# Illumina/Pisces

Measured on AMD Instinct MI355X. Metric: candidate loci/s at 500x depth, higher is better.
Workload: dtype int32 counts + f64 likelihoods; 1 GPU; BASELINE config 2: synthetic 100000 loci x 500x amplicon pileup, SNV-only, gVCF, per GPU per step; device-resident packed tuples; depth=500, ring_batches=6, tile_loci=56, parallelism=interval-shard x1

## Files before the change

### include/pisces_hip.h

```cpp
#ifndef PISCES_HIP_H
#define PISCES_HIP_H

#include <stdint.h>

#ifdef __cplusplus
extern "C" {
#endif

#define PISCES_HIP_ABI_VERSION 8

#define PISCES_OK                 0
#define PISCES_E_INVALID_ARG     -1
#define PISCES_E_BUFFER_TOO_SMALL -2
#define PISCES_E_DEVICE          -3
#define PISCES_E_UNMAPPED_BASE   -4
#define PISCES_E_UNSUPPORTED     -5
#define PISCES_E_STATE           -6
#define PISCES_E_INTERNAL        -7

enum { PISCES_ALLELE_A = 0, PISCES_ALLELE_G = 1, PISCES_ALLELE_C = 2, PISCES_ALLELE_T = 3,
       PISCES_ALLELE_N = 4, PISCES_ALLELE_DEL = 5, PISCES_NUM_ALLELE_TYPES = 6 };
enum { PISCES_DIR_FORWARD = 0, PISCES_DIR_REVERSE = 1, PISCES_DIR_STITCHED = 2, PISCES_NUM_DIRECTIONS = 3 };
enum { PISCES_CAT_SNV = 0, PISCES_CAT_INSERTION = 1, PISCES_CAT_DELETION = 2, PISCES_CAT_MNV = 3,
       PISCES_CAT_REFERENCE = 4 };
// ... 145 lines not shown
    const uint8_t* directions;
    const uint8_t* deletion_directions;
} PiscesReadBatch;
#define PISCES_DIR_UNTRACKED 255

typedef struct PiscesCandidate {
    int32_t position;
    int32_t category;
    int32_t ref_len, alt_len;
    int32_t support_by_dir[3];
    int32_t well_anchored_by_dir[3];
    uint8_t open_left, open_right;
    uint8_t pad[2];
    int64_t allele_offset;
} PiscesCandidate;

typedef struct PiscesHip PiscesHip;

int32_t pisces_hip_default_config(PiscesHipConfig* cfg);
int32_t pisces_hip_create(const PiscesHipConfig* cfg, int32_t device, PiscesHip** out);
int32_t pisces_hip_device_count(void);
int32_t pisces_hip_destroy(PiscesHip* h);
int64_t pisces_hip_trim_memory(void);
const char* pisces_hip_last_error(const PiscesHip* h);
int32_t pisces_hip_abi_version(void);

int32_t pisces_hip_set_reference(PiscesHip* h, const uint8_t* upper_bases, int64_t length);

int32_t pisces_hip_set_intervals(PiscesHip* h, const int32_t* starts, const int32_t* ends, int32_t n);

int32_t pisces_hip_set_owned_range(PiscesHip* h, int32_t lo, int32_t hi);

int32_t pisces_hip_add_reads(PiscesHip* h, const PiscesReadBatch* batch);
int32_t pisces_hip_stage_reads(PiscesHip* h, int32_t n_reads, int64_t n_cigar_ops, int64_t n_bases, int32_t with_directions,
                               int32_t with_deletion_directions, PiscesReadBatch* views);
int32_t pisces_hip_add_device_reads(PiscesHip* h, const PiscesReadBatch* device_batch, int64_t n_cigar_ops, int64_t n_bases);
int32_t pisces_hip_add_observations(PiscesHip* h, const int32_t* positions, const uint32_t* tuples, int64_t n);
int32_t pisces_hip_flush(PiscesHip* h, int32_t up_to_position, PiscesCalledAllele* out,
                         int64_t capacity, int64_t* n_out);
int32_t pisces_hip_flush_ex(PiscesHip* h, int32_t up_to_position, PiscesCalledAllele* out, int64_t capacity, int64_t* n_out,
                            int32_t* cand_index_out, PiscesCandidate* cand_out, int64_t cand_capacity, int64_t* n_cand,
                            uint8_t* alleles_out, int64_t allele_capacity, int64_t* allele_bytes);
int32_t pisces_hip_flush_begin(PiscesHip* h, int32_t up_to_position);
int32_t pisces_hip_flush_end(PiscesHip* h, PiscesCalledAllele* out, int64_t capacity, int64_t* n_out);
int32_t pisces_hip_flush_end_ex(PiscesHip* h, PiscesCalledAllele* out, int64_t capacity, int64_t* n_out, int32_t* cand_index_out,
                                PiscesCandidate* cand_out, int64_t cand_capacity, int64_t* n_cand, uint8_t* alleles_out,
// ... 194 lines not shown
```

### pisces_amd/_native.py

```python
import ctypes as C
import os

from . import _abi

_HERE = os.path.dirname(os.path.abspath(__file__))
LIB_PATH = os.environ.get("PISCES_HIP_LIB") or os.path.join(_HERE, "libpisceship.so")

EXPORTS = [
    "pisces_hip_abi_version", "pisces_hip_default_config", "pisces_hip_create", "pisces_hip_destroy", "pisces_hip_trim_memory",
    "pisces_hip_last_error", "pisces_hip_set_reference", "pisces_hip_set_intervals", "pisces_hip_add_reads", "pisces_hip_stage_reads", "pisces_hip_flush_begin", "pisces_hip_flush_end",
    "pisces_hip_add_observations", "pisces_hip_flush", "pisces_hip_get_counts", "pisces_hip_add_gapped_mnv_ref",
    "pisces_hip_get_candidates", "pisces_hip_stats", "pisces_hip_call_tiles", "pisces_hip_accumulate_tiles",
    "pisces_hip_synchronize", "pisces_hip_last_kernel_ms", "pisces_hip_expand_reads", "pisces_hip_device_totals",
    "pisces_hip_set_timing", "pisces_hip_kernel_time", "pisces_hip_set_chain_timing", "pisces_hip_chain_time", "pisces_hip_flush_ex", "pisces_hip_probe_read_bandwidth",
    "pisces_hip_vcf_default_config", "pisces_hip_format_vcf", "pisces_hip_format_vcf_padded", "pisces_hip_find_candidates", "pisces_hip_call_tiles_batched",
    "pisces_hip_find_indel_candidates", "pisces_hip_compact_records", "pisces_hip_bgzf_scan", "pisces_hip_bgzf_inflate",
    "pisces_hip_balanced_tile_loci", "pisces_hip_bam_decode", "pisces_hip_bam_fetch", "pisces_hip_bam_chain_mode", "pisces_hip_add_decoded_reads", "pisces_hip_find_candidates_device", "pisces_hip_get_base_quality_sums", "pisces_hip_get_gapped_mnv_ref", "pisces_hip_comm_unique_id", "pisces_hip_comm_init", "pisces_hip_reduce_summary", "pisces_hip_comm_destroy",
    "pisces_hip_add_candidates", "pisces_hip_set_forced_alleles", "pisces_hip_host_time", "pisces_hip_set_owned_range", "pisces_hip_bam_fetch_directions", "pisces_hip_call_tiles_graph_build", "pisces_hip_call_tiles_graph_launch", "pisces_hip_mark", "pisces_hip_marked_ms",
    "pisces_hip_flush_end_ex", "pisces_hip_device_count", "pisces_hip_flush_view", "pisces_hip_flush_end_view", "pisces_hip_transfer_bytes",
    "pisces_hip_add_device_reads", "pisces_hip_get_stream", "pisces_hip_comm_library", "pisces_hip_comm_ranks", "pisces_hip_set_known_variants", "pisces_hip_set_exclude_mnvs_from_collapsing", "pisces_hip_set_exact_total_called", "pisces_hip_reallocate_failed_mnvs", "pisces_hip_set_genotypes", "pisces_hip_diploid_genotype_qscore",
    "pisces_hip_adaptive_default_params", "pisces_hip_set_adaptive_params", "pisces_hip_get_posteriors", "pisces_hip_posteriors_view", "pisces_hip_set_posteriors_buffer",
    "pisces_hip_compact_posteriors", "pisces_hip_set_genotypes_adaptive", "pisces_hip_adaptive_genotype_qscore", "pisces_hip_format_vcf_ex", "pisces_hip_format_vcf_padded_ex",
    "pisces_hip_amplicon_bias", "pisces_hip_set_amplicon_bias_filter", "pisces_hip_add_reads_amplicons", "pisces_hip_add_device_reads_amplicons",
    "pisces_hip_get_amplicon_counts", "pisces_hip_bam_fetch_amplicons", "pisces_hip_amplicon_name_count", "pisces_hip_get_amplicon_name",
    "pisces_hip_intern_amplicon_name",
    "pisces_hip_exact_span_direction", "pisces_hip_set_coverage_method", "pisces_hip_get_spanning_read_counts",
    "pisces_hip_format_vcf_device",
]


class PiscesHipError(RuntimeError):
    def __init__(self, code, message):
# ... 7 lines not shown
    spec = importlib.util.find_spec("torch")
    if spec is None or not spec.origin:
        return
    cand = os.path.join(os.path.dirname(spec.origin), "lib", "libamdhip64.so")
    if os.path.exists(cand):
        C.CDLL(cand, mode=C.RTLD_GLOBAL)


def _load():
    _share_hip_runtime_with_torch()
    if not os.path.exists(LIB_PATH):
        raise ImportError(
            f"{LIB_PATH} is missing: the HIP extension has not been built. Run `python -c 'import __graft_entry__ as g; "
            "g.build()'` (needs hipcc). pisces_amd has no CPU fallback.")
    lib = C.CDLL(LIB_PATH)
    i32, i64, vp = C.c_int32, C.c_int64, C.c_void_p
    P = C.POINTER
    sig = {
        "pisces_hip_abi_version": (i32, []),
        "pisces_hip_default_config": (i32, [P(_abi.PiscesHipConfig)]),
        "pisces_hip_create": (i32, [P(_abi.PiscesHipConfig), i32, P(vp)]),
        "pisces_hip_destroy": (i32, [vp]),
        "pisces_hip_trim_memory": (C.c_int64, []),
        "pisces_hip_last_error": (C.c_char_p, [vp]),
        "pisces_hip_set_reference": (i32, [vp, vp, i64]),
        "pisces_hip_set_intervals": (i32, [vp, vp, vp, i32]),
        "pisces_hip_add_reads": (i32, [vp, P(_abi.PiscesReadBatch)]),
        "pisces_hip_add_device_reads": (i32, [vp, P(_abi.PiscesReadBatch), i64, i64]),
        "pisces_hip_reallocate_failed_mnvs": (i32, [vp, i64, vp, i64, vp, i64, i32, vp, i64, P(i64), vp, i64, P(i64), vp, i64, P(i64)]),
        "pisces_hip_set_genotypes": (i32, [P(_abi.PiscesHipConfig), P(_abi.PiscesGenotypeAllele), i32, vp, i64]),
        "pisces_hip_diploid_genotype_qscore": (i32, [i32, i32, i32, i32, i32]),
        "pisces_hip_adaptive_default_params": (i32, [P(_abi.PiscesAdaptiveParams)]),
        "pisces_hip_set_adaptive_params": (i32, [vp, P(_abi.PiscesAdaptiveParams)]),
        "pisces_hip_get_posteriors": (i32, [vp, vp, i64, P(i64)]),
        "pisces_hip_posteriors_view": (i32, [vp, P(vp), P(i64)]),
        "pisces_hip_set_posteriors_buffer": (i32, [vp, vp, i64]),
        "pisces_hip_compact_posteriors": (i32, [vp, vp, vp, i32, vp, vp, i32, vp]),
        "pisces_hip_set_genotypes_adaptive": (i32, [P(_abi.PiscesHipConfig), P(_abi.PiscesAdaptiveParams), P(_abi.PiscesGenotypeAllele), i32, vp, i64, vp]),
        "pisces_hip_adaptive_genotype_qscore": (i32, [P(_abi.PiscesAdaptiveParams), i32, i32, i32, i32, P(i32), P(i32), P(C.c_float)]),
        "pisces_hip_amplicon_bias": (i32, [P(i32), P(i32), i32, C.c_float, P(C.c_double)]),
        "pisces_hip_set_amplicon_bias_filter": (i32, [vp, C.c_float]),
        "pisces_hip_add_reads_amplicons": (i32, [vp, P(_abi.PiscesReadBatch), vp]),
        "pisces_hip_add_device_reads_amplicons": (i32, [vp, P(_abi.PiscesReadBatch), i64, i64, vp]),
        "pisces_hip_get_amplicon_counts": (i32, [vp, i32, i32, vp, vp, vp]),
        "pisces_hip_stage_reads": (i32, [vp, i32, i64, i64, i32, i32, P(_abi.PiscesReadBatch)]),
        "pisces_hip_flush_begin": (i32, [vp, i32]),
# ... 84 lines not shown
```

### pisces_amd/csrc/device_math.hip.h

```cpp
#pragma once
#include <hip/hip_runtime.h>
#include <stdint.h>

#include "../../include/pisces_hip.h"
#include "poisson_core.h"

namespace pisces {

struct DeviceParams {
    int32_t min_bq, noise_level, max_vq, min_vq, vq_filter, min_cov, low_depth_filter;
    int32_t min_gq, max_gq, low_gq_filter, sb_model, filter_single_strand, include_ref, emit_zero_cov;
    int32_t rmxn_max_len, rmxn_min_rep;
    float min_freq, vf_filter, gt_min_freq, target_lod, nocall_thr, rmxn_freq_limit;
    double sb_threshold;
    double err_q;
    double err_sb;
    double ln10;
    unsigned long long* totals;
    const double* q_to_p_lut;
    int32_t q_to_p_n;
    const double* gq_tail;
    int32_t gq_tail_a, gq_tail_cov;
    int32_t refs_only;
    int32_t variants_only;
    const int16_t* vq_tab;
    const double* sb_tab;
    const double* sb0_tab;
    const int16_t* gq_cap;
    int32_t vq_tab_k, sb_tab_k, tab_cov;
    const uint32_t* dirty_bits;
    int32_t dirty_first, dirty_n;
    int32_t* folded_out;
    int32_t folded_first, folded_n;
};

__device__ __forceinline__ bool locus_is_dirty(const DeviceParams& P, int pos)
{
    if (!P.dirty_bits) return false;
    const unsigned rel = (unsigned)(pos - P.dirty_first);
    return rel < (unsigned)P.dirty_n && ((P.dirty_bits[rel >> 5] >> (rel & 31u)) & 1u) != 0u;
}


__device__ __forceinline__ double ln_lower_bound(double r) { return (double)ilogb(r) * 0.6931471805; }

__device__ inline double poisson_cdf_sb(double num_occurrences, double expected)
{
    const double a = (double)(int)(num_occurrences + 1.0), x = expected;
    if (x > 0.0 && a >= 1.0 && 2.0 * x <= a) {
        const double r = a / x;
        if (a * (ln_lower_bound(r) - 1.0) + x > 51.0) return 1.0;
        if (a * (log(r) - 1.0) + x > 51.0) return 1.0;
    }
    return incomplete_gamma_function(a, x);
}


// ... 406 lines not shown
        if (nonAlleleObservationsF >= expectedNonAllelObservationsF) { gq = P.min_gq; return true; }
        return false;
    }
    double qScore = fmin((double)P.max_gq, (double)variantQ);
    qScore = fmax(qScore, (double)P.min_gq);
    gq = (int32_t)rint(qScore);
    return true;
}

struct AlleleTables {
    int32_t vq;
    double sb[3];
    int32_t gq_cap;
    int32_t gq_idx;
    uint32_t have;
};
__device__ __forceinline__ bool tables_complete(const DeviceParams& P) { return P.vq_tab && P.sb_tab && P.sb0_tab && P.gq_cap; }

__device__ __forceinline__ AlleleTables request_allele_tables(bool isRef, int32_t support, int32_t total, int32_t refsup, const int32_t cov[3],
                                                              const int32_t sup[3], const DeviceParams& P)
{
    AlleleTables t;
    const uint32_t tab_cov = (uint32_t)P.tab_cov;
    const bool vq_in = support > 0 && total > 0 && support < P.vq_tab_k && total < P.tab_cov;
    const int16_t vq_v = P.vq_tab[vq_in ? (uint32_t)support * tab_cov + (uint32_t)total : 0u];
    const int s2 = sup[2] / 2, c2 = cov[2] / 2;
    const int ss[3] = {sup[0] + sup[1] + sup[2], sup[0] + s2, sup[1] + s2};
    const int cc[3] = {cov[0] + cov[1] + cov[2], cov[0] + c2, cov[1] + c2};
    double sb_v[3];
    uint32_t have = vq_in ? 1u : 0u;
#pragma unroll
    for (int w = 0; w < 3; w++) {
        const bool zero = ss[w] == 0;
        const bool in = zero ? (P.sb_model != PISCES_SB_POISSON && cc[w] >= 0 && cc[w] < P.tab_cov)
                             : (ss[w] > 0 && ss[w] < P.sb_tab_k && cc[w] >= 0 && cc[w] < P.tab_cov);
        const double* base = zero ? P.sb0_tab : P.sb_tab;
        const uint32_t idx = in ? (zero ? (uint32_t)cc[w] : (uint32_t)ss[w] * tab_cov + (uint32_t)cc[w]) : 0u;
        sb_v[w] = base[idx];
        have |= in ? (2u << w) : 0u;
    }
    t.gq_idx = somatic_gq_index(somatic_genotype(isRef, total, support, refsup, P), total, support, P);
    const int16_t gq_v = P.gq_cap[t.gq_idx >= 0 ? t.gq_idx : 0];
    t.vq = vq_v;
    t.sb[0] = sb_v[0]; t.sb[1] = sb_v[1]; t.sb[2] = sb_v[2];
    t.gq_cap = gq_v;
    t.have = have;
    return t;
}

__device__ __forceinline__ bool poisson_qscore_try(int32_t callCount, int32_t coverage, const DeviceParams& P, const AlleleTables& t, int32_t& vq)
{
    if ((callCount <= 0) || (coverage <= 0)) { vq = 0; return true; }
    if (t.have & 1u) { vq = t.vq; return true; }
    const double lambda = P.err_q * coverage;
    if (P.max_vq <= 110 && callCount >= 3 && (double)callCount >= 2.0 * lambda) {
        const double km1 = callCount - 1;
        const double need = ((double)P.max_vq + 1.0) * 0.23025850929940458 + 1e-3;
        if (km1 * (ln_ratio_lower_bound(km1, lambda) - 1.0) >= need) { vq = P.max_vq; return true; }
    }
    return false;
}

__device__ __forceinline__ bool sb_stats_try(int32_t support, int32_t coverage, const DeviceParams& P, bool have, double value, SbStats& st)
{
    st.support = (double)support;
    st.coverage = (double)coverage;
    if (support == 0) {
        if (P.sb_model == PISCES_SB_POISSON) {
            st.false_pos = 1;
            st.var_gt_zero = 0;
            return true;
        }
        if (!have) return false;
        st.var_gt_zero = value;
        st.false_pos = 1 - st.var_gt_zero;
        return true;
    }
    if (have) {
        st.var_gt_zero = value;
    } else {
        const double a = (double)support, x = (double)coverage * P.err_sb;
        if (!(x > 0.0 && 2.0 * x <= a && a * (ln_ratio_lower_bound(a, x) - 1.0) + x > 51.0)) return false;
        st.var_gt_zero = 1.0;
    }
    st.false_pos = fmax(0.0, 1 - st.var_gt_zero);
    return true;
}

__device__ __forceinline__ bool strand_bias_try(const int32_t cov[3], const int32_t sup[3], const DeviceParams& P, const AlleleTables& t,
                                                double& bias_score, int& acceptable, int& var_both, int& cov_both)
{
    const int s2 = sup[2] / 2, c2 = cov[2] / 2;
    const int sf = sup[0] + s2, sr = sup[1] + s2, cf = cov[0] + c2, cr = cov[1] + c2;
    SbStats overall, fwd, rev;
    const bool ok0 = sb_stats_try(sup[0] + sup[1] + sup[2], cov[0] + cov[1] + cov[2], P, (t.have & 2u) != 0, t.sb[0], overall);
    const bool ok1 = sb_stats_try(sf, cf, P, (t.have & 4u) != 0, t.sb[1], fwd);
    const bool ok2 = sb_stats_try(sr, cr, P, (t.have & 8u) != 0, t.sb[2], rev);
    double forwardBias = 0.0, reverseBias = 0.0;
    if (!(fwd.false_pos == 0.0 && rev.false_pos == 0.0 && overall.var_gt_zero > 0.0)) {
        forwardBias = (fwd.var_gt_zero * rev.false_pos) / overall.var_gt_zero;
        reverseBias = (rev.var_gt_zero * fwd.false_pos) / overall.var_gt_zero;
        if (overall.var_gt_zero == 0) {
            forwardBias = 1;
            reverseBias = 1;
        }
    }
    double score = forwardBias > reverseBias ? forwardBias : reverseBias;
    cov_both = (cf > 0) && (cr > 0);
    var_both = (sf > 0) && (sr > 0);
    if (!cov_both) score = 0;
    bias_score = score;
    acceptable = score < P.sb_threshold;
    return ok0 && ok1 && ok2;
}

__device__ __noinline__ int32_t poisson_qscore_out_of_line(int32_t callCount, int32_t coverage, double err, int32_t max_vq, double ln10)
{
    const QParams q = {max_vq, ln10};
    return poisson_qscore_core(callCount, coverage, err, q);
}
// ... 80 lines not shown
```

### pisces_amd/csrc/kernels.hip.h

```cpp
#pragma once
#include <hip/hip_runtime.h>
#include <stdint.h>

#include "device_math.hip.h"
#include "genotype_core.h"

namespace pisces {

constexpr int kBlock = 256;
constexpr int kTile = 64;
constexpr int kFolded = 18;
constexpr int kUnroll = 8;
constexpr int kSlotsPerTile = 4 * kTile;
#ifndef PISCES_TOTAL_SHARDS
#define PISCES_TOTAL_SHARDS 64
#endif
constexpr int kTotalShards = PISCES_TOTAL_SHARDS;
constexpr int kTotalStride = 16;
constexpr int kRefMargin = 32;
constexpr int kRefWin = kTile + 2 * kRefMargin;
constexpr int kWaveRows = 32;
constexpr int kWaveRow = kTile;
constexpr int kWaveRegion = kWaveRows * kWaveRow;
constexpr int kQLutLds = 128;
// ... 707 lines not shown
__global__ __launch_bounds__(256) void build_vq_tab_kernel(int16_t* __restrict__ tab, int32_t n_k, int32_t n_cov, DeviceParams P)
{
    const int64_t i = (int64_t)blockIdx.x * blockDim.x + threadIdx.x;
    if (i >= (int64_t)n_k * n_cov) return;
    tab[i] = (int16_t)poisson_qscore((int32_t)(i / n_cov), (int32_t)(i % n_cov), P);
}
__global__ __launch_bounds__(256) void build_sb_tab_kernel(double* __restrict__ tab, double* __restrict__ tab0, int32_t n_k, int32_t n_cov, DeviceParams P)
{
    const int64_t i = (int64_t)blockIdx.x * blockDim.x + threadIdx.x;
    if (i >= (int64_t)n_k * n_cov) return;
    const int k = (int)(i / n_cov), cov = (int)(i % n_cov);
    tab[i] = k >= 1 ? fmax(0.0, poisson_cdf_sb((double)k - 1, (double)cov * P.err_sb)) : 0.0;
    if (k == 0) tab0[cov] = pow(1 - P.err_sb, (double)cov);
}
__global__ __launch_bounds__(256) void build_gq_cap_kernel(int16_t* __restrict__ tab, const double* __restrict__ gq_tail, int32_t n_a, int32_t n_cov, DeviceParams P)
{
    const int64_t i = (int64_t)blockIdx.x * blockDim.x + threadIdx.x;
    if (i >= (int64_t)n_a * n_cov) return;
    if (i < n_cov) { tab[i] = 0; return; }
    double rawQ = p_to_q(q_to_p_int(P.max_vq, P) + gq_tail[i]);
    double qScore = fmin((double)P.max_gq, rawQ);
    qScore = fmax(qScore, (double)P.min_gq);
    tab[i] = (int16_t)rint(qScore);
}

__global__ __launch_bounds__(64) void totals_collect_kernel(unsigned long long* __restrict__ shards, unsigned long long* __restrict__ out_host, int reset)
{
    const int l = threadIdx.x;
    if (l < 4) {
        unsigned long long v = 0;
        for (int sh = 0; sh < kTotalShards; sh++) v += shards[sh * kTotalStride + l];
        out_host[l] = v;
    }
    if (reset)
        for (int i = l; i < kTotalShards * kTotalStride; i += 64) shards[i] = 0ull;
    __threadfence_system();
}

__global__ __launch_bounds__(256) void read_probe_kernel(const u32x4* __restrict__ p, int64_t n4, uint32_t* __restrict__ sink)
{
    uint32_t acc = 0;
    const int64_t stride = (int64_t)gridDim.x * blockDim.x * 8;
    for (int64_t i = (int64_t)blockIdx.x * blockDim.x * 8 + threadIdx.x; i < n4; i += stride) {
        u32x4 v[8];
#pragma unroll
        for (int u = 0; u < 8; u++) {
// ... 808 lines not shown
```

### pisces_amd/csrc/pisces_hip.hip

```cpp
#include <hip/hip_runtime.h>
#include <hip/hip_ext.h>
#include <dlfcn.h>
#include <link.h>

#include <algorithm>
#include <array>
#include <cctype>
#include <memory>
#include <cmath>
#include <cstdio>
#include <cstdlib>
#include <cstring>
#include <deque>
#include <ctime>
#include <map>
#include <set>
#include <string>
#include <atomic>
#include <chrono>
#include <mutex>
#include <thread>
#include <unordered_map>
#include <unordered_set>
#include <vector>
// ... 263 lines not shown
    std::unordered_map<std::string, int32_t> amp_name_id;
    bool exact_on = false;
    bool exact_l0_set = false;
    DeviceBuf<int32_t> d_exact_words;
    DeviceBuf<int32_t> d_exact_extra, d_exact_spans, d_exact_out;
    DeviceBuf<PiscesTile> d_tiles_x;
    DeviceBuf<PiscesTileResult> d_tr_x;
    DeviceBuf<PiscesCalledAllele> d_rec_x;
    DeviceBuf<int32_t> d_cnt_x, d_off_x;
    int32_t* h_cnt_x = nullptr;
    bool tables_shareable = false;
    bool poisoned = false;
    std::string poison_why;
    uint8_t* h_prep = nullptr;
    DeviceBuf<double> d_qlut;
    DeviceBuf<ulonglong2> d_bq_lut;
    DeviceBuf<unsigned long long> d_sumq_fix;
    DeviceBuf<double> d_sumq;
    DeviceBuf<double> d_gq_tail;
    DeviceBuf<int16_t> d_vq_tab;
    DeviceBuf<double> d_sb_tab;
    DeviceBuf<double> d_sb0_tab;
    DeviceBuf<int16_t> d_gq_cap;
    DeviceBuf<DeviceParams> d_params;
    int n_cus = 256;
    void* comm = nullptr;
    int comm_world = 1;
    DeviceBuf<long long> d_summary;
    DeviceBuf<int32_t> d_offsets;
    DeviceBuf<PiscesCalledAllele> d_compact;
    DeviceBuf<PiscesGenotypePosteriors> d_post, d_post_compact;
    int kernel_variant = 4;
    std::string err;

    DeviceBuf<uint8_t> d_ref;
    std::vector<uint8_t> h_ref;
    int64_t ref_len = 0;
    DeviceBuf<DevCandidate> d_cands;
    DeviceBuf<uint8_t> d_alleles;
    DeviceBuf<PiscesCalledAllele> d_cand_records;
    DeviceBuf<uint8_t> d_cand_callable;
    int32_t* h_counts = nullptr;
    size_t h_counts_cap = 0;

    std::map<int32_t, BlockObs> blocks;
    int32_t last_block_key_cache = 0;
// ... 313 lines not shown
    P.min_bq = c.min_base_call_quality;
    P.noise_level = c.noise_level;
    P.max_vq = c.max_variant_qscore;
    P.min_vq = c.min_variant_qscore;
    P.vq_filter = c.variant_qscore_filter;
    P.min_cov = c.min_coverage;
    P.low_depth_filter = c.low_depth_filter;
    P.min_gq = c.min_genotype_qscore;
    P.max_gq = c.max_genotype_qscore;
    P.low_gq_filter = c.low_gq_filter;
    P.sb_model = c.strand_bias_model;
    P.filter_single_strand = c.filter_single_strand;
    P.include_ref = c.include_reference_calls;
    P.emit_zero_cov = c.emit_zero_coverage_refs;
    P.rmxn_max_len = c.rmxn_max_repeat_length;
    P.rmxn_min_rep = c.rmxn_min_repetitions;
    P.min_freq = c.min_frequency;
    P.vf_filter = c.variant_freq_filter;
    P.gt_min_freq = c.genotype_min_freq_filter;
    P.target_lod = c.target_lod_frequency;
    P.nocall_thr = c.no_call_filter_threshold;
    P.rmxn_freq_limit = c.rmxn_frequency_limit;
    P.sb_threshold = (double)c.strand_bias_threshold;
    P.err_q = std::pow(10.0, -1 * (double)c.noise_level / 10.0);
    P.err_sb = std::pow(10.0, (double)((float)(-1 * c.noise_level) / 10.0f));
    P.ln10 = std::log(10.0);
    P.totals = nullptr;
    P.q_to_p_lut = nullptr;
    P.q_to_p_n = 0;
    P.gq_tail = nullptr;
    P.gq_tail_a = 0;
    P.gq_tail_cov = 0;
    P.refs_only = c.call_mnvs ? 1 : 0;
    P.variants_only = 0;
    P.vq_tab = nullptr;
    P.sb_tab = nullptr;
    P.sb0_tab = nullptr;
    P.gq_cap = nullptr;
    P.vq_tab_k = P.sb_tab_k = P.tab_cov = 0;
    P.dirty_bits = nullptr;
    P.dirty_first = P.dirty_n = 0;
    P.folded_out = nullptr;
    P.folded_first = P.folded_n = 0;
    return P;
}

template <typename R, typename F>
static R abi_guard(PiscesHip* h, F&& body)
{
    try {
        return body();
    } catch (const std::exception& e) {
        return (R)fail(h, PISCES_E_INTERNAL, std::string("exception inside the library: ") + e.what());
    } catch (...) {
        return (R)fail(h, PISCES_E_INTERNAL, "unknown exception inside the library");
    }
}

namespace {
struct TableSet {
    PiscesHipConfig cfg;
    int device = 0;
    DeviceBuf<double> gq_tail, sb_tab, sb0_tab;
    DeviceBuf<int16_t> vq_tab, gq_cap;
};
std::mutex g_tables_mu;
std::vector<TableSet*>& table_cache() { static std::vector<TableSet*>* v = new std::vector<TableSet*>(); return *v; }
TableSet* take_tables(const PiscesHipConfig& cfg, int device)
{
    std::lock_guard<std::mutex> lock(g_tables_mu);
    auto& v = table_cache();
    for (size_t i = 0; i < v.size(); i++)
        if (v[i]->device == device && std::memcmp(&v[i]->cfg, &cfg, sizeof(cfg)) == 0) {
            TableSet* t = v[i];
            v.erase(v.begin() + (std::ptrdiff_t)i);
            return t;
        }
    return nullptr;
}
void leave_tables(TableSet* t)
{
    std::lock_guard<std::mutex> lock(g_tables_mu);
    auto& v = table_cache();
    v.push_back(t);
    if (v.size() > 8) { delete v.front(); v.erase(v.begin()); }
}
}

// ... 131 lines not shown
        if ((e = h->d_qlut.reserve((size_t)n)) != hipSuccess ||
            (e = hipMemcpy(h->d_qlut.p, lut.data(), (size_t)n * sizeof(double), hipMemcpyHostToDevice)) != hipSuccess) {
            g_create_error = std::string("pisces_hip_create: ") + hipGetErrorString(e);
            pisces_hip_destroy(h);
            return PISCES_E_DEVICE;
        }
        h->P.q_to_p_lut = h->d_qlut.p;
        h->P.q_to_p_n = n;
    }
    if (h->cfg.noise_model == PISCES_NOISE_WINDOW) {
        if ((e = ensure_quality_lut(h)) != hipSuccess) {
            g_create_error = std::string("pisces_hip_create: ") + hipGetErrorString(e);
            pisces_hip_destroy(h);
            return PISCES_E_DEVICE;
        }
    }
    if ((e = h->d_log_n.reserve(4)) != hipSuccess || (e = h->d_flags.reserve(4)) != hipSuccess ||
        (e = hipMemset(h->d_log_n.p, 0, 4 * sizeof(unsigned long long))) != hipSuccess ||
        (e = hipMemset(h->d_flags.p, 0, 4 * sizeof(int32_t))) != hipSuccess) {
        g_create_error = std::string("pisces_hip_create: ") + hipGetErrorString(e);
        pisces_hip_destroy(h);
        return PISCES_E_DEVICE;
    }
    const bool tables_by_default = !getenv("PISCES_HIP_NO_GQ_TABLE") && !getenv("PISCES_HIP_NO_CALL_TABLES") && h->cfg.noise_model == PISCES_NOISE_FLAT &&
                                   h->cfg.strand_bias_model != PISCES_SB_DIPLOID && h->cfg.max_variant_qscore <= 32767 && h->cfg.max_genotype_qscore <= 32767 &&
                                   h->cfg.min_genotype_qscore >= -32768;
    std::unique_ptr<TableSet> kept(tables_by_default ? take_tables(h->cfg, h->device) : nullptr);
    if (kept) {
        h->d_gq_tail.swap(kept->gq_tail); h->d_vq_tab.swap(kept->vq_tab); h->d_sb_tab.swap(kept->sb_tab); h->d_sb0_tab.swap(kept->sb0_tab); h->d_gq_cap.swap(kept->gq_cap);
        h->P.gq_tail = h->d_gq_tail.p; h->P.gq_tail_a = 32; h->P.gq_tail_cov = 8192;
        h->P.vq_tab = h->d_vq_tab.p; h->P.sb_tab = h->d_sb_tab.p; h->P.sb0_tab = h->d_sb0_tab.p; h->P.gq_cap = h->d_gq_cap.p;
        h->P.vq_tab_k = h->P.sb_tab_k = 256;
        h->P.tab_cov = 8192;
        h->tables_shareable = true;
    }
    if (!kept && !getenv("PISCES_HIP_NO_GQ_TABLE")) {
        const int32_t n_a = 32, n_cov = 8192;
        if ((e = h->d_gq_tail.reserve((size_t)n_a * n_cov)) != hipSuccess) {
            g_create_error = std::string("pisces_hip_create: ") + hipGetErrorString(e);
            pisces_hip_destroy(h);
            return PISCES_E_DEVICE;
        }
        hipLaunchKernelGGL(build_gq_tail_kernel, dim3((unsigned)((n_a * n_cov + 255) / 256)), dim3(256), 0, h->stream, h->d_gq_tail.p,
                           n_a, n_cov, h->P.target_lod);
        if ((e = hipGetLastError()) != hipSuccess || (e = hipStreamSynchronize(h->stream)) != hipSuccess) {
            g_create_error = std::string("pisces_hip_create: ") + hipGetErrorString(e);
            pisces_hip_destroy(h);
            return PISCES_E_DEVICE;
        }
        h->P.gq_tail = h->d_gq_tail.p;
        h->P.gq_tail_a = n_a;
        h->P.gq_tail_cov = n_cov;
    }
    if (!kept && !getenv("PISCES_HIP_NO_CALL_TABLES") && h->cfg.noise_model == PISCES_NOISE_FLAT && h->cfg.strand_bias_model != PISCES_SB_DIPLOID &&
        h->cfg.max_variant_qscore <= 32767 && h->cfg.max_genotype_qscore <= 32767 && h->cfg.min_genotype_qscore >= -32768) {
        const int32_t n_k = 256, n_cov = 8192;
        if ((e = h->d_vq_tab.reserve((size_t)n_k * n_cov)) != hipSuccess || (e = h->d_sb_tab.reserve((size_t)n_k * n_cov)) != hipSuccess ||
            (e = h->d_sb0_tab.reserve((size_t)n_cov)) != hipSuccess ||
            (h->P.gq_tail && (e = h->d_gq_cap.reserve((size_t)h->P.gq_tail_a * h->P.gq_tail_cov)) != hipSuccess)) {
            g_create_error = std::string("pisces_hip_create: ") + hipGetErrorString(e);
            pisces_hip_destroy(h);
            return PISCES_E_DEVICE;
        }
        const unsigned nb = (unsigned)(((size_t)n_k * n_cov + 255) / 256);
        hipLaunchKernelGGL(build_vq_tab_kernel, dim3(nb), dim3(256), 0, h->stream, h->d_vq_tab.p, n_k, n_cov, h->P);
        hipLaunchKernelGGL(build_sb_tab_kernel, dim3(nb), dim3(256), 0, h->stream, h->d_sb_tab.p, h->d_sb0_tab.p, n_k, n_cov, h->P);
        if (h->P.gq_tail)
            hipLaunchKernelGGL(build_gq_cap_kernel, dim3((unsigned)((h->P.gq_tail_a * h->P.gq_tail_cov + 255) / 256)), dim3(256), 0, h->stream,
                               h->d_gq_cap.p, h->P.gq_tail, h->P.gq_tail_a, h->P.gq_tail_cov, h->P);
        if ((e = hipGetLastError()) != hipSuccess || (e = hipStreamSynchronize(h->stream)) != hipSuccess) {
            g_create_error = std::string("pisces_hip_create: ") + hipGetErrorString(e);
            pisces_hip_destroy(h);
            return PISCES_E_DEVICE;
        }
        h->P.vq_tab = h->d_vq_tab.p;
        h->P.sb_tab = h->d_sb_tab.p;
        h->P.sb0_tab = h->d_sb0_tab.p;
        h->P.gq_cap = h->P.gq_tail ? h->d_gq_cap.p : nullptr;
        h->P.vq_tab_k = h->P.sb_tab_k = n_k;
        h->P.tab_cov = n_cov;
        h->tables_shareable = tables_by_default && h->P.gq_tail != nullptr;
    }
    if ((e = h->d_params.reserve(1)) != hipSuccess || (e = hipMemcpy(h->d_params.p, &h->P, sizeof(DeviceParams), hipMemcpyHostToDevice)) != hipSuccess) {
        g_create_error = std::string("pisces_hip_create: ") + hipGetErrorString(e);
        pisces_hip_destroy(h);
        return PISCES_E_DEVICE;
    }
    *out = h;
    return PISCES_OK;
    });
}

int64_t pisces_hip_trim_memory(void)
{
    {
        std::lock_guard<std::mutex> lock(g_tables_mu);
        for (TableSet* t : table_cache()) delete t;
        table_cache().clear();
    }
    AllocCache& c = alloc_cache();
    std::lock_guard<std::mutex> lock(c.m);
    int dev = 0;
    (void)hipGetDevice(&dev);
    const size_t freed = cache_drop(c, -2);
    (void)hipSetDevice(dev);
    return (int64_t)freed;
}

int32_t pisces_hip_destroy(PiscesHip* h)
{
    return abi_guard<int32_t>(h, [&]() -> int32_t {
    if (!h) return PISCES_OK;
    if (h->prof_on) {
        static const char* names[19] = {"consume_found", "spanning: candidates of the batch", "spanning: counts to the host", "collapse", "device pass (MNVs)",
                                        "reallocate", "device pass (all)", "call_blocks", "row merge / genotypers", "copy out + DoneProcessing", "split: dirty loci + SNV store", "  of reallocate: mnv_reallocate_failed",
                                        "add_device_reads: consume_found", "add_device_reads: copies + checks", "add_device_reads: shape + discovery + commit",
                                        "add_reads: place + reserve", "add_reads: staging + upload", "add_reads: pass over the CIGARs", "add_reads: launches + commit"};
        for (int i = 0; i < 19; i++) fprintf(stderr, "pisces_hip host profile: %-36s %9.3f ms\n", names[i], h->prof[i] * 1e3);
        if (h->mnv_split)
            fprintf(stderr, "pisces_hip split form: %lld SNV groups into the store, %lld taken by flushes (dirty loci), %lld dropped unseen, %lld sweeps\n",
                    (long long)h->split_stats[0], (long long)h->split_stats[1], (long long)h->split_stats[2], (long long)h->split_stats[3]);
    }
    (void)hipSetDevice(h->device);
    bool idle = !h->stream || hipStreamSynchronize(h->stream) == hipSuccess;
    for (int k = 0; k < PiscesHip::kLanes; k++)
        if (h->lane[k] && hipStreamSynchronize(h->lane[k]) != hipSuccess) idle = false;
    if (h->foreign_stream_ever && hipDeviceSynchronize() != hipSuccess) idle = false;
    (void)pisces_hip_comm_destroy(h);
    struct KeepFreed {
        explicit KeepFreed(bool on) { tl_keep_freed = on; }
        ~KeepFreed() { tl_keep_freed = false; }
    } keep(idle);
    if (idle && h->tables_shareable && h->d_vq_tab.p && h->d_gq_tail.p && h->d_gq_cap.p) {
        TableSet* t = new TableSet();
        t->cfg = h->cfg;
        t->device = h->device;
        t->gq_tail.swap(h->d_gq_tail); t->vq_tab.swap(h->d_vq_tab); t->sb_tab.swap(h->d_sb_tab); t->sb0_tab.swap(h->d_sb0_tab); t->gq_cap.swap(h->d_gq_cap);
        leave_tables(t);
    }
    h->d_summary.release();
    h->d_ref.release(); h->d_tuples.release(); h->d_tiles.release(); h->d_tile_results.release();
    h->d_records.release(); h->d_counts.release(); h->d_gapped.release(); h->d_count.release(); h->d_totals.release(); h->d_qlut.release(); h->d_bq_lut.release(); h->d_sumq_fix.release(); h->d_sumq.release(); h->d_gq_tail.release(); h->d_vq_tab.release(); h->d_sb_tab.release(); h->d_sb0_tab.release(); h->d_gq_cap.release(); h->d_params.release(); h->d_offsets.release(); h->d_compact.release(); h->d_post.release(); h->d_post_compact.release();
    for (int i = 0; i < 2; i++) { h->d_log_pos[i].release(); h->d_log_tup[i].release(); }
    h->d_log_n.release(); h->d_flags.release(); h->d_bucket.release(); h->d_total.release();
    for (auto& st : h->stage) {
        st.d.release();
        if (st.h) host_free(st.h);
        st.h = nullptr;
        if (st.done) (void)hipEventDestroy(st.done);
        st.done = nullptr;
    }
    h->h_stage = nullptr;
    if (h->async.done) (void)hipEventDestroy(h->async.done);
    h->async.done = nullptr;
    if (h->h_dl) host_free(h->h_dl);
    h->h_dl = nullptr;
    if (h->h_post) host_free(h->h_post);
    h->h_post = nullptr;
    if (h->h_cand_dl) host_free(h->h_cand_dl);
    h->h_cand_dl = nullptr;
    if (h->h_meta) host_free(h->h_meta);
    h->h_meta = nullptr;
    if (h->h_counts) host_free(h->h_counts);
    h->h_counts = nullptr;
    if (h->found.h) host_free(h->found.h);
// ... 137 lines not shown
```

### pisces_amd/engine.py

```python
import ctypes as C

import numpy as np

from . import _abi
from ._native import PiscesHipError, lib


def _check(handle, rc):
    if rc != 0:
        msg = lib.pisces_hip_last_error(handle)
        raise PiscesHipError(rc, msg.decode() if msg else "")


class DeviceReadBatch:

    def __init__(self, position, flags, cigar_offset, cigar_op, cigar_len, seq_offset, bases, quals, directions=None, deletion_directions=None,
                 n_ops=None, n_bases=None):
        import torch
        self.torch = torch
        self.tensors = dict(position=position, flags=flags, cigar_offset=cigar_offset, cigar_op=cigar_op, cigar_len=cigar_len, seq_offset=seq_offset,
                            bases=bases, quals=quals, directions=directions, deletion_directions=deletion_directions)
        for k, t in self.tensors.items():
            assert t is None or (t.is_cuda and t.is_contiguous()), k
        self.n_reads = int(position.numel())
# ... 484 lines not shown
                                                                 ptr(d_cands), ptr(d_alleles), ptr(d_gp), text.data_ptr(), cap, ptr(offs),
                                                                 size_word.data_ptr(), ts.cuda_stream))
                ts.synchronize()
                need = int(size_word[0])
                if need < 0:
                    raise PiscesHipError(need, "format_vcf_device: a row the host formatter refuses too (a filter bit whose name the configuration "
                                               "does not give, or a candidate index without candidates)")
                if need <= cap:
                    break
                cap = need
            out = bytes(text[:need].cpu().numpy().tobytes())
            if line_offsets:
                written = offs.cpu().numpy()
                return out, written[written >= 0]
            return out

    def accumulate_tiles(self, d_tuples, d_tiles, n_tiles, d_counts, stream=None):
        _check(self._h, lib.pisces_hip_accumulate_tiles(self._h, d_tuples, d_tiles, n_tiles, d_counts, self._stream_arg(stream)))

    def device_totals(self, reset=False):
        s = (C.c_int64 * 4)()
        _check(self._h, lib.pisces_hip_device_totals(self._h, s, 1 if reset else 0))
        return {"records": s[0], "candidate_loci": s[1], "called": s[2], "tiles": s[3]}

    def mark(self, which, stream=None):
        _check(self._h, lib.pisces_hip_mark(self._h, int(which), self._stream_arg(stream)))

    def marked_ms(self):
        ms = C.c_float(0)
        _check(self._h, lib.pisces_hip_marked_ms(self._h, C.byref(ms)))
        return ms.value

    def set_timing(self, enable=True):
        _check(self._h, lib.pisces_hip_set_timing(self._h, int(enable)))

    def kernel_time(self):
        ms, n = C.c_double(0), C.c_int64(0)
        _check(self._h, lib.pisces_hip_kernel_time(self._h, C.byref(ms), C.byref(n)))
        return ms.value, n.value

    def SetChainTiming(self, enable=True):
        _check(self._h, lib.pisces_hip_set_chain_timing(self._h, int(bool(enable))))

    def ChainTime(self):
        out = (C.c_double * 2)()
        _check(self._h, lib.pisces_hip_chain_time(self._h, out))
# ... 312 lines not shown
```

Before: 2.551 billion candidate loci/s.

## Precompute per-coverage saturation thresholds to skip VQ/SB table lookups for reference calls

Builds two per-coverage threshold rows at create time: the smallest support at which the Poisson variant qscore saturates at max_vq, and the smallest at which the strand-bias false-positive probability reaches one. At call time, reference-allele loci compare support against these rows and global bounds, so they can skip the 2D vq/sb double-table gathers and the strand-bias arithmetic. The cost is extra create-time kernel work, a host readback, and small uint16 lookups. Correctness rests on the thresholds being monotone in support, which the host-side bound computation tries to guard.

```diff
diff --git a/include/pisces_hip.h b/include/pisces_hip.h
--- a/include/pisces_hip.h
+++ b/include/pisces_hip.h
@@ -191,6 +191,7 @@
 int32_t pisces_hip_device_count(void);
 int32_t pisces_hip_destroy(PiscesHip* h);
 int64_t pisces_hip_trim_memory(void);
+int32_t pisces_hip_threshold_rows(PiscesHip* h, uint16_t* sb_one_k, uint16_t* vq_cap_k, int32_t capacity, int32_t bounds[4]);
 const char* pisces_hip_last_error(const PiscesHip* h);
 int32_t pisces_hip_abi_version(void);
 
diff --git a/pisces_amd/_native.py b/pisces_amd/_native.py
--- a/pisces_amd/_native.py
+++ b/pisces_amd/_native.py
@@ -7,7 +7,7 @@
 LIB_PATH = os.environ.get("PISCES_HIP_LIB") or os.path.join(_HERE, "libpisceship.so")
 
 EXPORTS = [
-    "pisces_hip_abi_version", "pisces_hip_default_config", "pisces_hip_create", "pisces_hip_destroy", "pisces_hip_trim_memory",
+    "pisces_hip_abi_version", "pisces_hip_default_config", "pisces_hip_create", "pisces_hip_destroy", "pisces_hip_trim_memory", "pisces_hip_threshold_rows",
     "pisces_hip_last_error", "pisces_hip_set_reference", "pisces_hip_set_intervals", "pisces_hip_add_reads", "pisces_hip_stage_reads", "pisces_hip_flush_begin", "pisces_hip_flush_end",
     "pisces_hip_add_observations", "pisces_hip_flush", "pisces_hip_get_counts", "pisces_hip_add_gapped_mnv_ref",
     "pisces_hip_get_candidates", "pisces_hip_stats", "pisces_hip_call_tiles", "pisces_hip_accumulate_tiles",
@@ -61,6 +61,7 @@
         "pisces_hip_create": (i32, [P(_abi.PiscesHipConfig), i32, P(vp)]),
         "pisces_hip_destroy": (i32, [vp]),
         "pisces_hip_trim_memory": (C.c_int64, []),
+        "pisces_hip_threshold_rows": (i32, [vp, vp, vp, i32, vp]),
         "pisces_hip_last_error": (C.c_char_p, [vp]),
         "pisces_hip_set_reference": (i32, [vp, vp, i64]),
         "pisces_hip_set_intervals": (i32, [vp, vp, vp, i32]),
diff --git a/pisces_amd/csrc/device_math.hip.h b/pisces_amd/csrc/device_math.hip.h
--- a/pisces_amd/csrc/device_math.hip.h
+++ b/pisces_amd/csrc/device_math.hip.h
@@ -28,11 +28,18 @@
     const double* sb0_tab;
     const int16_t* gq_cap;
     int32_t vq_tab_k, sb_tab_k, tab_cov;
+    const uint16_t* sb_one_k;
+    const uint16_t* vq_cap_k;
+    int32_t sb_row_lo, sb_row_hi, vq_row_lo, vq_row_hi;
+    int32_t sb_zero_ok;
     const uint32_t* dirty_bits;
     int32_t dirty_first, dirty_n;
     int32_t* folded_out;
     int32_t folded_first, folded_n;
 };
+
+constexpr uint16_t kNoThreshold = 0xFFFFu;
+constexpr int32_t kNoRowBound = 0x7FFFFFFF;
 
 __device__ __forceinline__ bool locus_is_dirty(const DeviceParams& P, int pos)
 {
@@ -485,25 +492,56 @@
 {
     AlleleTables t;
     const uint32_t tab_cov = (uint32_t)P.tab_cov;
-    const bool vq_in = support > 0 && total > 0 && support < P.vq_tab_k && total < P.tab_cov;
-    const int16_t vq_v = P.vq_tab[vq_in ? (uint32_t)support * tab_cov + (uint32_t)total : 0u];
     const int s2 = sup[2] / 2, c2 = cov[2] / 2;
     const int ss[3] = {sup[0] + sup[1] + sup[2], sup[0] + s2, sup[1] + s2};
     const int cc[3] = {cov[0] + cov[1] + cov[2], cov[0] + c2, cov[1] + c2};
-    double sb_v[3];
-    uint32_t have = vq_in ? 1u : 0u;
+    const bool rows = isRef && P.sb_one_k != nullptr && P.vq_cap_k != nullptr;
+    const bool vq_range = rows && support > 0 && support <= total && total < P.tab_cov;
+    const bool vq_sure = vq_range && support >= P.vq_row_hi;
+    const bool vq_maybe = vq_range && !vq_sure && support >= P.vq_row_lo;
+    bool sb_sure[3], sb_maybe[3];
+    bool any_maybe = vq_maybe;
+#pragma unroll
+    for (int w = 0; w < 3; w++) {
+        const bool range = rows && ss[w] > 0 && ss[w] <= cc[w] && cc[w] < P.tab_cov;
+        sb_sure[w] = range && ss[w] >= P.sb_row_hi;
+        sb_maybe[w] = range && !sb_sure[w] && ss[w] >= P.sb_row_lo;
+        any_maybe = any_maybe || sb_maybe[w];
+    }
+    uint16_t vq_thr = kNoThreshold, sb_thr[3] = {kNoThreshold, kNoThreshold, kNoThreshold};
+    if (any_maybe) {
+        vq_thr = P.vq_cap_k[vq_maybe ? (uint32_t)total : 0u];
+#pragma unroll
+        for (int w = 0; w < 3; w++) sb_thr[w] = P.sb_one_k[sb_maybe[w] ? (uint32_t)cc[w] : 0u];
+    }
+    t.gq_idx = somatic_gq_index(somatic_genotype(isRef, total, support, refsup, P), total, support, P);
+    const int16_t gq_v = P.gq_cap[t.gq_idx >= 0 ? t.gq_idx : 0];
+    const bool vq_in = !vq_sure && support > 0 && total > 0 && support < P.vq_tab_k && total < P.tab_cov;
+    bool sb_in[3];
+    uint32_t want = vq_in ? 1u : 0u;
 #pragma unroll
     for (int w = 0; w < 3; w++) {
         const bool zero = ss[w] == 0;
-        const bool in = zero ? (P.sb_model != PISCES_SB_POISSON && cc[w] >= 0 && cc[w] < P.tab_cov)
-                             : (ss[w] > 0 && ss[w] < P.sb_tab_k && cc[w] >= 0 && cc[w] < P.tab_cov);
-        const double* base = zero ? P.sb0_tab : P.sb_tab;
-        const uint32_t idx = in ? (zero ? (uint32_t)cc[w] : (uint32_t)ss[w] * tab_cov + (uint32_t)cc[w]) : 0u;
-        sb_v[w] = base[idx];
-        have |= in ? (2u << w) : 0u;
-    }
-    t.gq_idx = somatic_gq_index(somatic_genotype(isRef, total, support, refsup, P), total, support, P);
-    const int16_t gq_v = P.gq_cap[t.gq_idx >= 0 ? t.gq_idx : 0];
+        sb_in[w] = !sb_sure[w] && (zero ? (P.sb_model != PISCES_SB_POISSON && cc[w] >= 0 && cc[w] < P.tab_cov)
+                                        : (ss[w] > 0 && ss[w] < P.sb_tab_k && cc[w] >= 0 && cc[w] < P.tab_cov));
+        want |= sb_in[w] ? (2u << w) : 0u;
+    }
+    int16_t vq_v = 0;
+    double sb_v[3] = {0.0, 0.0, 0.0};
+    if (want != 0u) {
+        vq_v = P.vq_tab[vq_in ? (uint32_t)support * tab_cov + (uint32_t)total : 0u];
+#pragma unroll
+        for (int w = 0; w < 3; w++) {
+            const bool zero = ss[w] == 0;
+            const double* base = zero ? P.sb0_tab : P.sb_tab;
+            const uint32_t idx = sb_in[w] ? (zero ? (uint32_t)cc[w] : (uint32_t)ss[w] * tab_cov + (uint32_t)cc[w]) : 0u;
+            sb_v[w] = base[idx];
+        }
+    }
+    uint32_t have = want;
+    have |= (vq_sure || (vq_maybe && support >= (int32_t)vq_thr)) ? 16u : 0u;
+#pragma unroll
+    for (int w = 0; w < 3; w++) have |= (sb_sure[w] || (sb_maybe[w] && ss[w] >= (int32_t)sb_thr[w])) ? (32u << w) : 0u;
     t.vq = vq_v;
     t.sb[0] = sb_v[0]; t.sb[1] = sb_v[1]; t.sb[2] = sb_v[2];
     t.gq_cap = gq_v;
@@ -514,6 +552,7 @@
 __device__ __forceinline__ bool poisson_qscore_try(int32_t callCount, int32_t coverage, const DeviceParams& P, const AlleleTables& t, int32_t& vq)
 {
     if ((callCount <= 0) || (coverage <= 0)) { vq = 0; return true; }
+    if (t.have & 16u) { vq = P.max_vq; return true; }
     if (t.have & 1u) { vq = t.vq; return true; }
     const double lambda = P.err_q * coverage;
     if (P.max_vq <= 110 && callCount >= 3 && (double)callCount >= 2.0 * lambda) {
@@ -524,10 +563,15 @@
     return false;
 }
 
-__device__ __forceinline__ bool sb_stats_try(int32_t support, int32_t coverage, const DeviceParams& P, bool have, double value, SbStats& st)
+__device__ __forceinline__ bool sb_stats_try(int32_t support, int32_t coverage, const DeviceParams& P, bool row, bool have, double value, SbStats& st)
 {
     st.support = (double)support;
     st.coverage = (double)coverage;
+    if (row) {
+        st.var_gt_zero = 1.0;
+        st.false_pos = 0.0;
+        return true;
+    }
     if (support == 0) {
         if (P.sb_model == PISCES_SB_POISSON) {
             st.false_pos = 1;
@@ -555,10 +599,17 @@
 {
     const int s2 = sup[2] / 2, c2 = cov[2] / 2;
     const int sf = sup[0] + s2, sr = sup[1] + s2, cf = cov[0] + c2, cr = cov[1] + c2;
+    if ((t.have & 0xE0u) == 0xE0u) {
+        cov_both = (cf > 0) && (cr > 0);
+        var_both = (sf > 0) && (sr > 0);
+        bias_score = 0.0;
+        acceptable = P.sb_zero_ok;
+        return true;
+    }
     SbStats overall, fwd, rev;
-    const bool ok0 = sb_stats_try(sup[0] + sup[1] + sup[2], cov[0] + cov[1] + cov[2], P, (t.have & 2u) != 0, t.sb[0], overall);
-    const bool ok1 = sb_stats_try(sf, cf, P, (t.have & 4u) != 0, t.sb[1], fwd);
-    const bool ok2 = sb_stats_try(sr, cr, P, (t.have & 8u) != 0, t.sb[2], rev);
+    const bool ok0 = sb_stats_try(sup[0] + sup[1] + sup[2], cov[0] + cov[1] + cov[2], P, (t.have & 32u) != 0, (t.have & 2u) != 0, t.sb[0], overall);
+    const bool ok1 = sb_stats_try(sf, cf, P, (t.have & 64u) != 0, (t.have & 4u) != 0, t.sb[1], fwd);
+    const bool ok2 = sb_stats_try(sr, cr, P, (t.have & 128u) != 0, (t.have & 8u) != 0, t.sb[2], rev);
     double forwardBias = 0.0, reverseBias = 0.0;
     if (!(fwd.false_pos == 0.0 && rev.false_pos == 0.0 && overall.var_gt_zero > 0.0)) {
         forwardBias = (fwd.var_gt_zero * rev.false_pos) / overall.var_gt_zero;
diff --git a/pisces_amd/csrc/kernels.hip.h b/pisces_amd/csrc/kernels.hip.h
--- a/pisces_amd/csrc/kernels.hip.h
+++ b/pisces_amd/csrc/kernels.hip.h
@@ -753,6 +753,30 @@
     double qScore = fmin((double)P.max_gq, rawQ);
     qScore = fmax(qScore, (double)P.min_gq);
     tab[i] = (int16_t)rint(qScore);
+}
+__global__ __launch_bounds__(64) void build_threshold_rows_kernel(uint16_t* __restrict__ sb_one_k, uint16_t* __restrict__ vq_cap_k, int32_t n_cov, DeviceParams P)
+{
+    const int cov = (int)blockIdx.x, lane = (int)threadIdx.x;
+    if (cov >= n_cov) return;
+    int sb_thr = 1, vq_thr = 1;
+    bool sb_open = true, vq_open = true;
+    for (int top = cov; top >= 1 && (sb_open || vq_open); top -= 64) {
+        const int k = top - lane;
+        if (sb_open) {
+            const bool fails = k >= 1 && !(fmax(0.0, poisson_cdf_sb((double)k - 1, (double)cov * P.err_sb)) == 1.0);
+            const unsigned long long m = __ballot(fails);
+            if (m) { sb_thr = top - (int)__builtin_ctzll(m) + 1; sb_open = false; }
+        }
+        if (vq_open) {
+            const bool fails = k >= 1 && poisson_qscore(k, cov, P) != P.max_vq;
+            const unsigned long long m = __ballot(fails);
+            if (m) { vq_thr = top - (int)__builtin_ctzll(m) + 1; vq_open = false; }
+        }
+    }
+    if (lane == 0) {
+        sb_one_k[cov] = sb_thr <= cov ? (uint16_t)sb_thr : kNoThreshold;
+        vq_cap_k[cov] = vq_thr <= cov ? (uint16_t)vq_thr : kNoThreshold;
+    }
 }
 
 __global__ __launch_bounds__(64) void totals_collect_kernel(unsigned long long* __restrict__ shards, unsigned long long* __restrict__ out_host, int reset)
diff --git a/pisces_amd/csrc/pisces_hip.hip b/pisces_amd/csrc/pisces_hip.hip
--- a/pisces_amd/csrc/pisces_hip.hip
+++ b/pisces_amd/csrc/pisces_hip.hip
@@ -309,6 +309,7 @@
     DeviceBuf<double> d_sb_tab;
     DeviceBuf<double> d_sb0_tab;
     DeviceBuf<int16_t> d_gq_cap;
+    DeviceBuf<uint16_t> d_sb_one_k, d_vq_cap_k;
     DeviceBuf<DeviceParams> d_params;
     int n_cus = 256;
     void* comm = nullptr;
@@ -668,6 +669,7 @@
     P.nocall_thr = c.no_call_filter_threshold;
     P.rmxn_freq_limit = c.rmxn_frequency_limit;
     P.sb_threshold = (double)c.strand_bias_threshold;
+    P.sb_zero_ok = 0.0 < P.sb_threshold ? 1 : 0;
     P.err_q = std::pow(10.0, -1 * (double)c.noise_level / 10.0);
     P.err_sb = std::pow(10.0, (double)((float)(-1 * c.noise_level) / 10.0f));
     P.ln10 = std::log(10.0);
@@ -683,6 +685,9 @@
     P.sb_tab = nullptr;
     P.sb0_tab = nullptr;
     P.gq_cap = nullptr;
+    P.sb_one_k = nullptr;
+    P.vq_cap_k = nullptr;
+    P.sb_row_lo = P.sb_row_hi = P.vq_row_lo = P.vq_row_hi = kNoRowBound;
     P.vq_tab_k = P.sb_tab_k = P.tab_cov = 0;
     P.dirty_bits = nullptr;
     P.dirty_first = P.dirty_n = 0;
@@ -709,7 +714,21 @@
     int device = 0;
     DeviceBuf<double> gq_tail, sb_tab, sb0_tab;
     DeviceBuf<int16_t> vq_tab, gq_cap;
+    DeviceBuf<uint16_t> sb_one_k, vq_cap_k;
+    int32_t row_bounds[4] = {0, 0, 0, 0};
 };
+void row_bounds(const uint16_t* row, int32_t n, int32_t& lo, int32_t& hi)
+{
+    lo = hi = kNoRowBound;
+    int32_t running_max = 0;
+    bool open = true;
+    for (int32_t k = n - 1; k >= 0; k--) {
+        if (row[k] != kNoThreshold && (int32_t)row[k] < lo) lo = row[k];
+        running_max = std::max(running_max, (int32_t)row[k]);
+        open = open && running_max <= k;
+        if (open) hi = k;
+    }
+}
 std::mutex g_tables_mu;
 std::vector<TableSet*>& table_cache() { static std::vector<TableSet*>* v = new std::vector<TableSet*>(); return *v; }
 TableSet* take_tables(const PiscesHipConfig& cfg, int device)
@@ -887,12 +906,16 @@
         pisces_hip_destroy(h);
         return PISCES_E_DEVICE;
     }
-    const bool tables_by_default = !getenv("PISCES_HIP_NO_GQ_TABLE") && !getenv("PISCES_HIP_NO_CALL_TABLES") && h->cfg.noise_model == PISCES_NOISE_FLAT &&
+    const bool threshold_rows = !getenv("PISCES_HIP_NO_THRESHOLD_ROWS");
+    const bool tables_by_default = !getenv("PISCES_HIP_NO_GQ_TABLE") && !getenv("PISCES_HIP_NO_CALL_TABLES") && threshold_rows && h->cfg.noise_model == PISCES_NOISE_FLAT &&
                                    h->cfg.strand_bias_model != PISCES_SB_DIPLOID && h->cfg.max_variant_qscore <= 32767 && h->cfg.max_genotype_qscore <= 32767 &&
                                    h->cfg.min_genotype_qscore >= -32768;
     std::unique_ptr<TableSet> kept(tables_by_default ? take_tables(h->cfg, h->device) : nullptr);
     if (kept) {
         h->d_gq_tail.swap(kept->gq_tail); h->d_vq_tab.swap(kept->vq_tab); h->d_sb_tab.swap(kept->sb_tab); h->d_sb0_tab.swap(kept->sb0_tab); h->d_gq_cap.swap(kept->gq_cap);
+        h->d_sb_one_k.swap(kept->sb_one_k); h->d_vq_cap_k.swap(kept->vq_cap_k);
+        h->P.sb_one_k = h->d_sb_one_k.p; h->P.vq_cap_k = h->d_vq_cap_k.p;
+        h->P.sb_row_lo = kept->row_bounds[0]; h->P.sb_row_hi = kept->row_bounds[1]; h->P.vq_row_lo = kept->row_bounds[2]; h->P.vq_row_hi = kept->row_bounds[3];
         h->P.gq_tail = h->d_gq_tail.p; h->P.gq_tail_a = 32; h->P.gq_tail_cov = 8192;
         h->P.vq_tab = h->d_vq_tab.p; h->P.sb_tab = h->d_sb_tab.p; h->P.sb0_tab = h->d_sb0_tab.p; h->P.gq_cap = h->d_gq_cap.p;
         h->P.vq_tab_k = h->P.sb_tab_k = 256;
@@ -922,6 +945,7 @@
         const int32_t n_k = 256, n_cov = 8192;
         if ((e = h->d_vq_tab.reserve((size_t)n_k * n_cov)) != hipSuccess || (e = h->d_sb_tab.reserve((size_t)n_k * n_cov)) != hipSuccess ||
             (e = h->d_sb0_tab.reserve((size_t)n_cov)) != hipSuccess ||
+            (threshold_rows && ((e = h->d_sb_one_k.reserve((size_t)n_cov)) != hipSuccess || (e = h->d_vq_cap_k.reserve((size_t)n_cov)) != hipSuccess)) ||
             (h->P.gq_tail && (e = h->d_gq_cap.reserve((size_t)h->P.gq_tail_a * h->P.gq_tail_cov)) != hipSuccess)) {
             g_create_error = std::string("pisces_hip_create: ") + hipGetErrorString(e);
             pisces_hip_destroy(h);
@@ -933,6 +957,8 @@
         if (h->P.gq_tail)
             hipLaunchKernelGGL(build_gq_cap_kernel, dim3((unsigned)((h->P.gq_tail_a * h->P.gq_tail_cov + 255) / 256)), dim3(256), 0, h->stream,
                                h->d_gq_cap.p, h->P.gq_tail, h->P.gq_tail_a, h->P.gq_tail_cov, h->P);
+        const bool rows = threshold_rows && h->P.gq_tail != nullptr;
+        if (rows) hipLaunchKernelGGL(build_threshold_rows_kernel, dim3((unsigned)n_cov), dim3(64), 0, h->stream, h->d_sb_one_k.p, h->d_vq_cap_k.p, n_cov, h->P);
         if ((e = hipGetLastError()) != hipSuccess || (e = hipStreamSynchronize(h->stream)) != hipSuccess) {
             g_create_error = std::string("pisces_hip_create: ") + hipGetErrorString(e);
             pisces_hip_destroy(h);
@@ -942,6 +968,19 @@
         h->P.sb_tab = h->d_sb_tab.p;
         h->P.sb0_tab = h->d_sb0_tab.p;
         h->P.gq_cap = h->P.gq_tail ? h->d_gq_cap.p : nullptr;
+        if (rows) {
+            std::vector<uint16_t> sb_row((size_t)n_cov), vq_row((size_t)n_cov);
+            if ((e = hipMemcpy(sb_row.data(), h->d_sb_one_k.p, (size_t)n_cov * sizeof(uint16_t), hipMemcpyDeviceToHost)) != hipSuccess ||
+                (e = hipMemcpy(vq_row.data(), h->d_vq_cap_k.p, (size_t)n_cov * sizeof(uint16_t), hipMemcpyDeviceToHost)) != hipSuccess) {
+                g_create_error = std::string("pisces_hip_create: ") + hipGetErrorString(e);
+                pisces_hip_destroy(h);
+                return PISCES_E_DEVICE;
+            }
+            row_bounds(sb_row.data(), n_cov, h->P.sb_row_lo, h->P.sb_row_hi);
+            row_bounds(vq_row.data(), n_cov, h->P.vq_row_lo, h->P.vq_row_hi);
+            h->P.sb_one_k = h->d_sb_one_k.p;
+            h->P.vq_cap_k = h->d_vq_cap_k.p;
+        }
         h->P.vq_tab_k = h->P.sb_tab_k = n_k;
         h->P.tab_cov = n_cov;
         h->tables_shareable = tables_by_default && h->P.gq_tail != nullptr;
@@ -970,6 +1009,22 @@
     const size_t freed = cache_drop(c, -2);
     (void)hipSetDevice(dev);
     return (int64_t)freed;
+}
+
+int32_t pisces_hip_threshold_rows(PiscesHip* h, uint16_t* sb_one_k, uint16_t* vq_cap_k, int32_t capacity, int32_t bounds[4])
+{
+    return abi_guard<int32_t>(h, [&]() -> int32_t {
+    if (!h || !sb_one_k || !vq_cap_k || capacity < 0) return fail(h, PISCES_E_INVALID_ARG, "pisces_hip_threshold_rows: null argument or negative capacity");
+    if (!h->P.sb_one_k || !h->P.vq_cap_k) return 0;
+    const int32_t n = h->P.tab_cov;
+    if (capacity < n) return fail(h, PISCES_E_INVALID_ARG, "pisces_hip_threshold_rows: capacity below the rows' length");
+    hipError_t e;
+    if ((e = hipSetDevice(h->device)) != hipSuccess || (e = hipMemcpy(sb_one_k, h->P.sb_one_k, (size_t)n * sizeof(uint16_t), hipMemcpyDeviceToHost)) != hipSuccess ||
+        (e = hipMemcpy(vq_cap_k, h->P.vq_cap_k, (size_t)n * sizeof(uint16_t), hipMemcpyDeviceToHost)) != hipSuccess)
+        return fail(h, PISCES_E_DEVICE, std::string("pisces_hip_threshold_rows: ") + hipGetErrorString(e));
+    if (bounds) { bounds[0] = h->P.sb_row_lo; bounds[1] = h->P.sb_row_hi; bounds[2] = h->P.vq_row_lo; bounds[3] = h->P.vq_row_hi; }
+    return n;
+    });
 }
 
 int32_t pisces_hip_destroy(PiscesHip* h)
@@ -996,16 +1051,18 @@
         explicit KeepFreed(bool on) { tl_keep_freed = on; }
         ~KeepFreed() { tl_keep_freed = false; }
     } keep(idle);
-    if (idle && h->tables_shareable && h->d_vq_tab.p && h->d_gq_tail.p && h->d_gq_cap.p) {
+    if (idle && h->tables_shareable && h->d_vq_tab.p && h->d_gq_tail.p && h->d_gq_cap.p && h->d_sb_one_k.p && h->d_vq_cap_k.p) {
         TableSet* t = new TableSet();
         t->cfg = h->cfg;
         t->device = h->device;
         t->gq_tail.swap(h->d_gq_tail); t->vq_tab.swap(h->d_vq_tab); t->sb_tab.swap(h->d_sb_tab); t->sb0_tab.swap(h->d_sb0_tab); t->gq_cap.swap(h->d_gq_cap);
+        t->sb_one_k.swap(h->d_sb_one_k); t->vq_cap_k.swap(h->d_vq_cap_k);
+        t->row_bounds[0] = h->P.sb_row_lo; t->row_bounds[1] = h->P.sb_row_hi; t->row_bounds[2] = h->P.vq_row_lo; t->row_bounds[3] = h->P.vq_row_hi;
         leave_tables(t);
     }
     h->d_summary.release();
     h->d_ref.release(); h->d_tuples.release(); h->d_tiles.release(); h->d_tile_results.release();
-    h->d_records.release(); h->d_counts.release(); h->d_gapped.release(); h->d_count.release(); h->d_totals.release(); h->d_qlut.release(); h->d_bq_lut.release(); h->d_sumq_fix.release(); h->d_sumq.release(); h->d_gq_tail.release(); h->d_vq_tab.release(); h->d_sb_tab.release(); h->d_sb0_tab.release(); h->d_gq_cap.release(); h->d_params.release(); h->d_offsets.release(); h->d_compact.release(); h->d_post.release(); h->d_post_compact.release();
+    h->d_records.release(); h->d_counts.release(); h->d_gapped.release(); h->d_count.release(); h->d_totals.release(); h->d_qlut.release(); h->d_bq_lut.release(); h->d_sumq_fix.release(); h->d_sumq.release(); h->d_gq_tail.release(); h->d_vq_tab.release(); h->d_sb_tab.release(); h->d_sb0_tab.release(); h->d_gq_cap.release(); h->d_sb_one_k.release(); h->d_vq_cap_k.release(); h->d_params.release(); h->d_offsets.release(); h->d_compact.release(); h->d_post.release(); h->d_post_compact.release();
     for (int i = 0; i < 2; i++) { h->d_log_pos[i].release(); h->d_log_tup[i].release(); }
     h->d_log_n.release(); h->d_flags.release(); h->d_bucket.release(); h->d_total.release();
     for (auto& st : h->stage) {
diff --git a/pisces_amd/engine.py b/pisces_amd/engine.py
--- a/pisces_amd/engine.py
+++ b/pisces_amd/engine.py
@@ -530,6 +530,14 @@
         s = (C.c_int64 * 4)()
         _check(self._h, lib.pisces_hip_device_totals(self._h, s, 1 if reset else 0))
         return {"records": s[0], "candidate_loci": s[1], "called": s[2], "tiles": s[3]}
+
+    def threshold_rows(self):
+        import numpy as np
+        sb, vq, bounds = np.zeros(1 << 16, np.uint16), np.zeros(1 << 16, np.uint16), np.zeros(4, np.int32)
+        n = lib.pisces_hip_threshold_rows(self._h, sb.ctypes.data, vq.ctypes.data, len(sb), bounds.ctypes.data)
+        if n < 0:
+            _check(self._h, n)
+        return (sb[:n].copy(), vq[:n].copy(), bounds) if n > 0 else None
 
     def mark(self, which, stream=None):
         _check(self._h, lib.pisces_hip_mark(self._h, int(which), self._stream_arg(stream)))
```

Measured after the change: 2.527 billion candidate loci/s. Within noise of the previous version (-1.0%).
